# lastz/lastz

Measured on AMD Instinct MI355X. Metric: Gbp-of-target aligned/sec (whole job, --nogapped HSP path, both strands), higher is better.
Workload: dtype s32

## Files before the change

lastz_amd/csrc/enum_kernels.hip:

```cpp
#include <hip/hip_runtime.h>
#include <algorithm>
#include <rocprim/device/device_radix_sort.hpp>
#include <rocprim/device/device_scan.hpp>
#include <rocprim/iterator/transform_iterator.hpp>
#include "lz_ctx.hpp"
#include "lz_host.hpp"
#include "lz_seed_dev.hpp"

__global__ void __launch_bounds__(LZ_TPB)
k_pack_words(const u8* __restrict__ qcode, u32 lo, u32 hi, LzSeedDev sd, u32* __restrict__ pk, u32* __restrict__ iv, u32 bshift, u32 kbits)
{
    __shared__ u8 win[LZ_TPB + 32];
    const u32 i = blockIdx.x * LZ_TPB + threadIdx.x;
    const u32 L = (u32)sd.length;
    const s64 first = (s64)lo + (s64)blockIdx.x * LZ_TPB + 1 - (s64)L;
    for (u32 k = threadIdx.x; k < LZ_TPB + L - 1; k += LZ_TPB) win[k] = (first + (s64)k < (s64)hi) ? qcode[first + (s64)k] : (u8)LZ_CODE_INVALID;
    __syncthreads();
    if (i < hi - lo) {
        const u32 pos2 = lo + i + 1;
        u64 w = 0; u32 bad = 0;
        for (u32 k = 0; k < L; k++) { const u32 c = win[threadIdx.x + k]; bad |= c; w = (w << 2) | LZ_CODE_BITS(c); }
        const bool valid = pos2 >= lo + L && !(bad & LZ_CODE_INVALID);
        pk[i] = ((i >> bshift) << kbits) | (valid ? lz_apply_seed(sd, w) : (1u << sd.weight));
        iv[i] = i;
    }
}
__global__ void k_block_starts(const u32* __restrict__ sk, u32 n, u32 kbits, u32 none, u32 nblk, u64* __restrict__ bs, u64* __restrict__ n_words)
{
    const u32 b = threadIdx.x;
    if (b > nblk) return;
    auto first_at_least = [&](u64 key) { u32 lo = 0, hi = n; while (lo < hi) { const u32 m = lo + ((hi - lo) >> 1); if ((u64)sk[m] < key) lo = m + 1; else hi = m; } return lo; };
    const u32 start = first_at_least((u64)b << kbits);
    bs[b] = start;
    if (b < nblk) atomicAdd((unsigned long long*)n_words, (unsigned long long)(first_at_least(((u64)b << kbits) | none) - start));
}

__global__ void __launch_bounds__(LZ_TPB)
k_count_sorted(const u32* __restrict__ sk, const u32* __restrict__ sv, u32 n, LzSeedDev sd,
               const u32* __restrict__ wstart, u32* __restrict__ cnt)
{
    const u32 j = blockIdx.x * LZ_TPB + threadIdx.x;
    if (j >= n) return;
    const u32 w0 = sk[j] & ((2u << sd.weight) - 1u);
    if (w0 >> sd.weight) return;
    u32 c = 0;
    for (int p = 0; p < sd.nprobes; p++) { const u32 w = w0 ^ sd.probe_xor[p]; c += wstart[w + 1] - wstart[w]; }
    cnt[sv[j]] = c;
}

__device__ __forceinline__ bool lz_owned(u32 pos1, u32 pos2, u32 n_owners, u32 owner)
{ return (((pos1 - pos2) & (LZ_DIAG_SIZE - 1)) % n_owners) == owner; }

__global__ void __launch_bounds__(LZ_TPB)
k_count_sorted_owned(const u32* __restrict__ sk, const u32* __restrict__ sv, u32 n, u32 lo, LzSeedDev sd,
                     const u32* __restrict__ wstart, const u32* __restrict__ wpos, u32* __restrict__ cnt,
                     u32 n_owners, u32 owner)
{
    const u32 j = blockIdx.x * LZ_TPB + threadIdx.x;
    if (j >= n) return;
    const u32 w0 = sk[j] & ((2u << sd.weight) - 1u);
    if (w0 >> sd.weight) return;
    const u32 i = sv[j], pos2 = lo + i + 1;
    u32 c = 0;
    for (int p = 0; p < sd.nprobes; p++) {
        const u32 w = w0 ^ sd.probe_xor[p];
        for (u32 k = wstart[w]; k < wstart[w + 1]; k++) c += lz_owned(wpos[k], pos2, n_owners, owner) ? 1u : 0u;
    }
    cnt[i] = c;
}

#define LZ_SELF_GROUP 16
__global__ void __launch_bounds__(LZ_TPB)
k_count_sorted_self(const u32* __restrict__ sk, const u32* __restrict__ sv, u32 n, u32 lo, LzSeedDev sd,
                    const u32* __restrict__ wstart, const u32* __restrict__ wpos, u32* __restrict__ cnt, LzSelfDev self)
{
    const u32 j = blockIdx.x * LZ_TPB + threadIdx.x;
    if (j >= n) return;
    const u32 w0 = sk[j] & ((2u << sd.weight) - 1u);
    if (w0 >> sd.weight) return;
    const u32 i = sv[j], pos2 = lo + i + 1;
    u32 blo, bhi;
    lz_self_bounds(self, pos2, blo, bhi);
    u32 c = 0;
    for (int r = 0; r < sd.nprobes; r += LZ_SELF_GROUP) {
        u32 a[LZ_SELF_GROUP], len[LZ_SELF_GROUP];
#pragma unroll
        for (int p = 0; p < LZ_SELF_GROUP; p++) {
            const bool on = r + p < sd.nprobes;
            const u32 w = on ? (w0 ^ sd.probe_xor[(r + p) & (LZ_MAX_PROBES - 1)]) : 0u;
            a[p] = wstart[w]; len[p] = wstart[w + 1];
        }
#pragma unroll
        for (int p = 0; p < LZ_SELF_GROUP; p++) { const bool on = r + p < sd.nprobes; len[p] = on ? len[p] - a[p] : 0u; }
        lz_clip_runs<LZ_SELF_GROUP>(wpos, a, len, blo, bhi);
#pragma unroll
        for (int p = 0; p < LZ_SELF_GROUP; p++) c += len[p];
    }
    cnt[i] = c;
}

int lzk_count_hits(LzCtx& c, const u8* qcode, u32 lo, u32 hi)
{
    const u32 n = hi - lo;
    u32* const cnt = c.cnt.as<u32>(); u32* const pk = c.pk.as<u32>(); u32* const iv = c.wiv.as<u32>();
    u32* const sk = c.wsk.as<u32>(); u32* const sv = c.wsv.as<u32>();
    LZ_HIP(hipMemsetAsync(cnt, 0, (size_t)n * 4, c.stream));
    const u32 kbits = (u32)c.seed.weight + 1u;
    const double est_hits = (double)n * (double)c.num_words * (double)c.seed.nprobes / (double)(1ull << c.seed.weight);
    u32 want_bits = 0;
    while (want_bits < 5 && est_hits > (double)c.hit_capacity * (double)(1u << want_bits) * 0.5) want_bits++;
    if (est_hits <= (double)c.hit_capacity) want_bits = 0;
    u32 bbits = std::min<u32>(want_bits, 32u - kbits);
    u32 bshift = 0;
    const u64 nm1 = n ? (u64)n - 1 : 0;
    while (bshift < 32 && (nm1 >> bshift) >= (1ull << bbits)) bshift++;
    c.blk_shift = bshift; c.blk_count = (u32)((nm1 >> bshift) + 1);
    c.timer.begin("k_pack_words", c.stream);
    hipLaunchKernelGGL(k_pack_words, dim3((n + LZ_TPB - 1) / LZ_TPB), dim3(LZ_TPB), 0, c.stream,
                       qcode, lo, hi, c.seed, pk, iv, bshift, kbits);
    c.timer.end(c.stream);
    LZ_HIP(hipGetLastError());
    size_t tmp = 0;
    const unsigned bits = kbits + bbits;
    LZ_HIP(rocprim::radix_sort_pairs(nullptr, tmp, pk, sk, iv, sv, (size_t)n, 0u, bits, c.stream));
    int rc = c.sort_tmp.ensure(tmp);
    if (rc) return rc;
    c.timer.begin("rocprim_sort_words", c.stream);
    LZ_HIP(rocprim::radix_sort_pairs(c.sort_tmp.p, tmp, pk, sk, iv, sv, (size_t)n, 0u, bits, c.stream));
    c.timer.end(c.stream);
    if ((rc = c.blk_start.ensure(130 * 8))) return rc;
    hipLaunchKernelGGL(k_block_starts, dim3(1), dim3(192), 0, c.stream, sk, n, kbits, 1u << c.seed.weight, c.blk_count, c.blk_start.as<u64>(), c.dev_counters.as<u64>() + 2);
    c.timer.begin("k_count_hits", c.stream);
    if (c.self.mode != LZ_SELF_OFF)
        hipLaunchKernelGGL(k_count_sorted_self, dim3((n + LZ_TPB - 1) / LZ_TPB), dim3(LZ_TPB), 0, c.stream,
                           sk, sv, n, lo, c.seed, c.wstart.as<u32>(), c.wpos.as<u32>(), cnt, c.self);
    else if (c.n_owners > 1)
        hipLaunchKernelGGL(k_count_sorted_owned, dim3((n + LZ_TPB - 1) / LZ_TPB), dim3(LZ_TPB), 0, c.stream,
                           sk, sv, n, lo, c.seed, c.wstart.as<u32>(), c.wpos.as<u32>(), cnt, c.n_owners, c.owner);
    else
        hipLaunchKernelGGL(k_count_sorted, dim3((n + LZ_TPB - 1) / LZ_TPB), dim3(LZ_TPB), 0, c.stream,
                           sk, sv, n, c.seed, c.wstart.as<u32>(), cnt);
    c.timer.end(c.stream);
    LZ_HIP(hipGetLastError());
    return 0;
}

struct U32ToU64 { __host__ __device__ u64 operator()(u32 x) const { return (u64)x; } };

int lzk_scan_counts(LzCtx& c, u32 n)
{
    const u32* const cnt = c.cnt.as<u32>(); u64* const off = c.off.as<u64>();
    auto in = rocprim::make_transform_iterator(cnt, U32ToU64());
    size_t tmp = 0;
    LZ_HIP(rocprim::exclusive_scan(nullptr, tmp, in, off, (u64)0, (size_t)n, rocprim::plus<u64>(), c.stream));
    int rc = c.scan_tmp.ensure(tmp);
    if (rc) return rc;
    c.timer.begin("rocprim_scan_counts", c.stream);
    LZ_HIP(rocprim::exclusive_scan(c.scan_tmp.p, tmp, in, off, (u64)0, (size_t)n, rocprim::plus<u64>(), c.stream));
    c.timer.end(c.stream);
    return 0;
}

__global__ void __launch_bounds__(LZ_TPB)
k_sample_offsets(const u64* __restrict__ off, const u32* __restrict__ cnt, u32 n, u32 stride, u32 ns, u64* __restrict__ out)
{
    const u32 k = blockIdx.x * LZ_TPB + threadIdx.x;
    if (k < ns) out[1 + k] = off[(size_t)k * stride];
    if (k == 0) out[0] = off[n - 1] + cnt[n - 1];
}

int lzk_sample_offsets(LzCtx& c, u32 n, u32 stride, u32 ns)
{
    hipLaunchKernelGGL(k_sample_offsets, dim3((ns + LZ_TPB - 1) / LZ_TPB), dim3(LZ_TPB), 0, c.stream, c.off.as<u64>(), c.cnt.as<u32>(), n, stride, ns, c.pinned);
    LZ_HIP(hipGetLastError());
    return 0;
}

__global__ void __launch_bounds__(LZ_TPB)
k_fill_hits(u32 lo, u32 i0, u32 i1, LzSeedDev sd,
            const u32* __restrict__ wstart, const u32* __restrict__ wpos,
            const u32* __restrict__ sk, const u32* __restrict__ sv, u32 n, const u64* __restrict__ off,
            u64 base, u64* __restrict__ keys, u32 n_owners, u32 owner)
{
    const u32 lane = threadIdx.x & 63u, p = lane & (LZ_FILL_GROUP - 1), g = lane >> 4;
    const u32 j = (blockIdx.x * LZ_TPB + threadIdx.x);
    u32 w_l = 0, i_l = 0; bool in = false;
    if (j < n) { w_l = sk[j] & ((2u << sd.weight) - 1u); i_l = sv[j]; in = !(w_l >> sd.weight) && i_l >= i0 && i_l < i1; }
    u64 todo = __ballot(in);
    while (todo) {
        int src = -1;
        u64 m = todo;
#pragma unroll
        for (int q = 0; q < 4; q++) {
            const int s_q = m ? (int)__ffsll((long long)m) - 1 : -1;
            if (m) m &= m - 1;
            if ((int)g == q) src = s_q;
        }
        todo = m;
        const bool have = src >= 0;
        const u32 packed = __shfl(w_l, have ? src : 0);
        const u32 i = __shfl(i_l, have ? src : 0);
        const u32 pos2 = lo + i + 1;
        u64* out = have ? keys + (off[i] - base) : keys;
        u32 carry = 0;
        for (int r = 0; r < sd.nprobes; r += LZ_FILL_GROUP) {
            u32 a = 0, len = 0, full = 0;
            if (have && r + (int)p < sd.nprobes) {
                const u32 w = packed ^ sd.probe_xor[r + p];
                a = wstart[w]; full = wstart[w + 1] - a;
                for (u32 jj = 0; jj < full; jj++) len += lz_owned(wpos[a + jj], pos2, n_owners, owner) ? 1u : 0u;
            }
            u32 incl = len;
#pragma unroll
            for (int d = 1; d < LZ_FILL_GROUP; d <<= 1) {
                u32 v = __shfl_up(incl, d, LZ_FILL_GROUP);
                if ((int)p >= d) incl += v;
            }
            const u32 total = __shfl(incl, LZ_FILL_GROUP - 1, LZ_FILL_GROUP);
            u64* o = out + carry + (incl - len);
            for (u32 jj = 0; jj < full; jj++) { const u32 p1 = wpos[a + jj]; if (lz_owned(p1, pos2, n_owners, owner)) *o++ = lz_hit_key(p1, pos2); }
            carry += total;
        }
    }
}

#define LZ_F2_CAP   2560
#define LZ_F2_WORDS (LZ_F2_CAP / 2 / 64)
template <bool SELF>
__global__ void __launch_bounds__(LZ_TPB)
k_fill_hits2(u32 lo, u32 i0, u32 i1, LzSeedDev sd,
             const u32* __restrict__ wstart, const u32* __restrict__ wpos,
             const u32* __restrict__ sk, const u32* __restrict__ sv, u32 n, const u64* __restrict__ off,
             u64 base, u64* __restrict__ keys, LzSelfDev self)
{
    __shared__ LzListWave<LZ_F2_CAP> shw[LZ_TPB / 64];
    LzListWave<LZ_F2_CAP>& sh = shw[threadIdx.x >> 6];
    unsigned short* const own = reinterpret_cast<unsigned short*>(sh.own32);
    const u32 lane = threadIdx.x & 63u;
    const u32 j = blockIdx.x * LZ_TPB + threadIdx.x;
    u32 w_l = 0, i_l = 0; bool in = false;
    if (j < n) { w_l = sk[j] & ((2u << sd.weight) - 1u); i_l = sv[j]; in = !(w_l >> sd.weight) && i_l >= i0 && i_l < i1; }
    if (!__ballot(in)) return;
    const u32 dbase = in ? (u32)(off[i_l] - base) : 0u;
    const u32 pos2 = lo + i_l + 1u;
    u32 slo = 0, shi = 0;
    if (SELF) lz_self_bounds(self, pos2, slo, shi);
    u32 carry = 0;
    for (int r = 0; r < sd.nprobes; r += LZ_FILL_GROUP) {
        u32 la[LZ_FILL_GROUP], len[LZ_FILL_GROUP]; u32 total = 0;
#pragma unroll
        for (int p = 0; p < LZ_FILL_GROUP; p++) {
            const bool on = in && r + p < sd.nprobes;
            const u32 w = on ? (w_l ^ sd.probe_xor[(r + p) & (LZ_MAX_PROBES - 1)]) : 0u;
            la[p] = wstart[w]; len[p] = wstart[w + 1];
        }
#pragma unroll
        for (int p = 0; p < LZ_FILL_GROUP; p++) {
            const bool on = in && r + p < sd.nprobes;
            len[p] = on ? len[p] - la[p] : 0u;
            if (!SELF) total += len[p];
        }
        if (SELF) {
            lz_clip_runs<LZ_FILL_GROUP>(wpos, la, len, slo, shi);
#pragma unroll
            for (int p = 0; p < LZ_FILL_GROUP; p++) total += len[p];
        }
        u32 inc = total;
        LZ_WAVE_SCAN_U32(inc, total, lz_uadd)
        const u32 E = inc - total;
        const u32 T = (u32)__builtin_amdgcn_readlane((int)inc, 63);
        {
            u32 S = E;
#pragma unroll
            for (int p = 0; p < LZ_FILL_GROUP; p++) { sh.lsrc[lane * LZ_FILL_GROUP + p] = la[p] - S; S += len[p]; }
        }
        sh.ent[lane] = make_uint2(dbase + carry - E, pos2);
        for (u32 cs = 0; cs < T; cs += LZ_F2_CAP) {
            const u32 tc = (T - cs < (u32)LZ_F2_CAP) ? T - cs : (u32)LZ_F2_CAP;
            uint4* const mine = reinterpret_cast<uint4*>(sh.own32 + lane * LZ_F2_WORDS);
#pragma unroll
            for (int k = 0; k < LZ_F2_WORDS / 4; k++) mine[k] = make_uint4(0u, 0u, 0u, 0u);
            __atomic_signal_fence(__ATOMIC_SEQ_CST);
            {
                u32 S = E;
#pragma unroll
                for (int p = 0; p < LZ_FILL_GROUP; p++) {
                    const u32 l = len[p];
                    if (l && S < cs + tc && S + l > cs) own[(S > cs ? S : cs) - cs] = (unsigned short)(1u + lane * LZ_FILL_GROUP + (u32)p);
                    S += l;
                }
            }
            __atomic_signal_fence(__ATOMIC_SEQ_CST);
            u32 wv[LZ_F2_WORDS];
#pragma unroll
// ... 61 lines not shown
```

lastz_amd/csrc/lz_ctx.hpp:

```cpp
#pragma once
#include <hip/hip_runtime.h>
#include <string>
#include <vector>
#include <map>
#include <mutex>
#include "lz_common.hpp"
#include "lz_settings.hpp"
#include "../../include/lzgpu.h"

struct DevBuf {
    void*  p = nullptr;
    size_t cap = 0;
    int ensure(size_t bytes);
    void release();
    template <class T> T* as() const { return (T*)p; }
};

struct KernelTimer {
    struct Pending { int id; hipEvent_t a, b; hipStream_t s; };
    bool enabled = false;
    std::vector<std::string> names;
    std::vector<uint64_t> launches;
    std::vector<double> ms;
    std::vector<Pending> pending;
    std::map<hipStream_t, std::vector<hipEvent_t>> pool;
    int  id_of(const char* name);
    void begin(const char* name, hipStream_t s);
    void end(hipStream_t s);
    void resolve();
    void reset();
    hipEvent_t get_event(hipStream_t s);
    int cur = -1; hipEvent_t cur_a = nullptr;
};

struct SeqSlot {
    DevBuf raw;
    DevBuf code;
    DevBuf dp;
    DevBuf nib;
    bool   have_nib = false;
    DevBuf two, spc;
    DevBuf two_x, spc_x;
    DevBuf occ_dev;
    u8     occ[256] = { 0 };
    bool   has_special = false;
    u32    len = 0;
    bool   have_raw = false;
    uint64_t code_key = 0;
    uint64_t dp_key = 0;
    std::vector<u8> host;
    u8* raw_base()  const { return raw.as<u8>()  + LZ_SEQ_PAD; }
    u8* code_base() const { return code.as<u8>() + LZ_SEQ_PAD; }
    void release()
    {
        DevBuf* all[] = { &raw, &code, &dp, &nib, &two, &spc, &two_x, &spc_x, &occ_dev };
        for (DevBuf* b : all) b->release();
        have_raw = have_nib = false; code_key = dp_key = 0;
    }
};

struct LzCtx {
    bool inited = false;
    int  device = -1;
    int  num_cus = 256;
    hipStream_t stream = nullptr;
    hipStream_t dp_stream = nullptr;
    std::string last_error;

    SeqSlot target;
    bool have_table = false;
    lz_table_geom geom;
    LzSeedDev seed;
    DevBuf wstart, wpos;
    u64 num_words = 0;
    u64 table_gen = 0;
    DevBuf wctx;
    u64 wctx_gen = 0; uint64_t wctx_code_key = 0;

    std::map<int, SeqSlot> queries;
#define LZ_TEMP_SLOT_B3 (-1000)
    std::mutex slots_m;

    DevBuf cnt, off, pk;
    DevBuf wiv, wsk, wsv;
    DevBuf blk_start;
    std::vector<u64> blk_start_host;
    u32 blk_shift = 0, blk_count = 1;
    u64* pinned = nullptr; size_t pinned_words = 0;
    DevBuf bins;
    DevBuf keys;
    DevBuf bin_base;
    DevBuf hist, hist_part, run_addr;
    DevBuf summ, scan_tasks, scan_ntasks;
    DevBuf lut;
    DevBuf sort_tmp, scan_tmp;
    DevBuf diag_end;
    DevBuf score_tab;
    std::vector<s32> score_sub;
    u8 rowc[256] = { 0 }, colc[256] = { 0 };
    std::vector<s32> lut_m4; s32 lut_xdrop = -1;
    DevBuf cls_t, cls_q, cls_tmp;
    DevBuf win_tab;
    DevBuf hsp_out, hsp_count;
    DevBuf hsp_mc;
    DevBuf dev_counters;
    DevBuf tb_keys, tb_vals, tb_keys2, tb_vals2;
    struct DpBufs { DevBuf jobs, ids, res, tab, tb, rows, ops, ops_off, ops_out, pieces, rings, sel_jobs, sel_res, problems; } dp;
    DevBuf win_jobs, win_scratch, win_out, win_count;
    bool win_attr_set = false;
    bool settle_attr_set = false;
    u64 dp_longest[4] = { 0, 0, 0, 0 };
    u32 dp_slot_tb = 8u << 20;
    u32 dp_window = 0;
    u32 n_owners = 1, owner = 0;
    LzSelfDev self = {};
    DevBuf self_sep;
    std::vector<u64> last_order;
    int min_scan_mode = 0;
    int last_scan_mode = -1;
    u64 hit_capacity = (1ull << 31);
    u64 hsp_capacity = (1ull << 24);

    lz_counters counters = {};
    std::mutex counters_m;
    KernelTimer timer;
    KernelTimer dp_timer;

    void release_device_memory()
    {
        DevBuf* all[] = { &wstart, &wpos, &wctx, &cnt, &off, &pk, &wiv, &wsk, &wsv, &blk_start, &bins, &keys, &bin_base, &hist, &hist_part, &run_addr,
                          &summ, &scan_tasks, &scan_ntasks, &lut, &sort_tmp, &scan_tmp, &diag_end, &score_tab, &cls_t, &cls_q, &cls_tmp, &win_tab,
                          &hsp_out, &hsp_count, &hsp_mc, &dev_counters, &tb_keys, &tb_vals, &tb_keys2, &tb_vals2, &self_sep,
                          &dp.jobs, &dp.ids, &dp.res, &dp.tab, &dp.tb, &dp.rows, &dp.ops, &dp.ops_off, &dp.ops_out, &dp.pieces, &dp.rings, &dp.sel_jobs, &dp.sel_res, &dp.problems,
                          &win_jobs, &win_scratch, &win_out, &win_count };
        for (DevBuf* b : all) b->release();
        target.release();
        for (auto& kv : queries) kv.second.release();
        queries.clear();
        if (pinned) (void)hipHostFree(pinned);
        pinned = nullptr; pinned_words = 0;
        have_table = false; wctx_gen = 0; wctx_code_key = 0;
        score_sub.clear(); lut_m4.clear(); lut_xdrop = -1;
        win_attr_set = false; settle_attr_set = false;
    }
};

LzCtx& lz_ctx();
int lz_bind_thread();
int lz_fail(int code, const char* fmt, ...);
#define LZ_HIP(expr) do { hipError_t _e = (expr); if (_e != hipSuccess) \
    return lz_fail(LZGPU_ERR_HIP, "%s:%d %s -> %s", __FILE__, __LINE__, #expr, hipGetErrorString(_e)); } while (0)

struct LzChunk; struct LzLutParams;
#include "lz_tile_runs.hpp"
int lzk_encode(LzCtx& c, const u8* raw, u8* code, u32 len, const u8* cls256_dev, hipStream_t st = nullptr, KernelTimer* timer = nullptr);
int lzk_pack_nibbles(LzCtx& c, const u8* code_alloc, u8* nib, size_t nbytes);
int lzk_pack2(LzCtx& c, const u8* code_base, const u8* raw_base, u32 len, u8* two, u8* spc, u32 nmask, u32* flags256);
int lzk_overlap32(LzCtx& c, const u8* src, u8* dst, size_t nblocks);
int lzk_table_build(LzCtx& c);
int lzk_table_export(LzCtx& c, u32* last_dev, u32* prev_dev, u32 prev_entries);
int lzk_wctx_build(LzCtx& c);
int lzk_count_hits(LzCtx& c, const u8* qcode, u32 lo, u32 hi);
int lzk_scan_counts(LzCtx& c, u32 n);
int lzk_sample_offsets(LzCtx& c, u32 n, u32 stride, u32 ns);
int lzk_fill_hits(LzCtx& c, u32 lo, const LzChunk& ch, u32 n);
int lzk_scan_reserve(LzCtx& c, int mode, u64 max_n);
int lzk_scan_hits(LzCtx& c, int mode, const LzExtendParams& P, const LzLutParams& Q, u64 n);
int lzk_fused_reserve(LzCtx& c, u64 max_n);
int lzk_scan_fused(LzCtx& c, u32 lo, const LzChunk& ch, u32 n, const LzExtendParams& P, const LzLutParams& Q);
int lzk_partition(LzCtx& c, bool tagged, u64 n);
int lzk_hist_scan(LzCtx& c, u64 n);
int lzk_settle(LzCtx& c, const LzExtendParams& P, u64 n, u32 out_cap);
int lzk_hsp_match_counts(LzCtx& c, u32 n_rec, const SeqSlot& q);
```

lastz_amd/csrc/lzgpu_api.hip:

```cpp
#include <hip/hip_runtime.h>
#include <stdarg.h>
#include <stdio.h>
#include <stdlib.h>
#include <string.h>
#include <math.h>
#include <algorithm>
#include <mutex>
#include <thread>
#include <atomic>
#include "lz_ctx.hpp"
#include "lz_host.hpp"
#include "lz_lut.hpp"


static LzCtx g_ctx;
void lz_phase_clocks_print();
LzCtx& lz_ctx() { return g_ctx; }

static thread_local std::string t_last_error, t_last_error_out;
static std::mutex g_err_m;
int lz_fail(int code, const char* fmt, ...)
{
    char buf[512];
    va_list ap; va_start(ap, fmt); vsnprintf(buf, sizeof(buf), fmt, ap); va_end(ap);
// ... 281 lines not shown
    memset(&c.geom, 0, sizeof(c.geom));
    c.geom.tlen = tlen; c.geom.start = start; c.geom.end = end; c.geom.step = step; c.geom.seed = *seed;
    memcpy(c.geom.char_to_bits, char_to_bits, 256);
    if ((rc = slot_upload(c, c.target, t, tlen, true))) return rc;
    u8 cls[256]; lzh_make_cls(nullptr, char_to_bits, cls);
    if ((rc = slot_encode(c, c.target, cls, c.cls_t))) return rc;
    if ((rc = lzk_table_build(c))) return rc;
    c.geom.num_words = c.num_words;
    c.have_table = true;
    return 0;
}

extern "C" int lzgpu_target_upload(const uint8_t* t, uint32_t tlen)
{
    int rc = require_init(); if (rc) return rc;
    LzCtx& c = g_ctx;
    if (!t) return lz_fail(LZGPU_ERR_ARG, "null argument");
    if (tlen >= 0x7FFFFFFFu) return LZGPU_NH_SIZE;
    c.have_table = false;
    memset(&c.geom, 0, sizeof(c.geom));
    c.geom.tlen = tlen;
    return slot_upload(c, c.target, t, tlen, true);
}

extern "C" int lzgpu_table_rebuild(void)
{
    LzCtx& c = g_ctx;
    if (!c.have_table) return lz_fail(LZGPU_ERR_STATE, "no position table");
    int rc = lz_bind_thread(); if (rc) return rc;
    rc = lzk_table_build(c);
    if (!rc) c.geom.num_words = c.num_words;
    return rc;
}

extern "C" uint64_t lzgpu_table_num_words(void) { return g_ctx.have_table ? g_ctx.num_words : 0; }

extern "C" int lzgpu_table_export(uint32_t* last, uint32_t* prev)
{
    LzCtx& c = g_ctx;
    if (!c.have_table) return lz_fail(LZGPU_ERR_STATE, "no position table");
    u32 nwords = 1u << c.seed.weight;
    u32 adj = c.geom.start - (c.geom.start % c.geom.step);
    u32 prev_entries = 1 + (c.geom.end - adj) / c.geom.step;
    DevBuf dl, dp; int rc;
    if ((rc = lz_bind_thread())) return rc;
    if (last && (rc = dl.ensure((size_t)nwords * 4))) return rc;
    if (prev && (rc = dp.ensure((size_t)prev_entries * 4))) { dl.release(); return rc; }
    rc = lzk_table_export(c, last ? dl.as<u32>() : nullptr, prev ? dp.as<u32>() : nullptr, prev_entries);
    if (!rc) {
        if (last) (void)hipMemcpyAsync(last, dl.p, (size_t)nwords * 4, hipMemcpyDeviceToHost, c.stream);
        if (prev) (void)hipMemcpyAsync(prev, dp.p, (size_t)prev_entries * 4, hipMemcpyDeviceToHost, c.stream);
        if (hipStreamSynchronize(c.stream) != hipSuccess) rc = lz_fail(LZGPU_ERR_HIP, "table export copy failed");
    }
    dl.release(); dp.release();
    return rc;
}

extern "C" int lzgpu_table_geom(lz_table_geom* out)
{
    if (!g_ctx.have_table || !out) return lz_fail(LZGPU_ERR_STATE, "no position table");
    *out = g_ctx.geom; return 0;
}

extern "C" int lzgpu_table_adopt(const lz_table_geom* g)
{
    int rc = require_init(); if (rc) return rc;
    LzCtx& c = g_ctx;
    if (!g) return LZGPU_ERR_ARG;
    if ((rc = lzh_seed_to_dev(&g->seed, c.seed))) return rc;
    c.have_table = false; c.geom = *g; c.num_words = g->num_words; c.table_gen++;
    size_t total = (size_t)g->tlen + 2 * LZ_SEQ_PAD + 16;
    if ((rc = c.target.raw.ensure(total))) return rc;
    if ((rc = c.target.code.ensure(total))) return rc;
    LZ_HIP(hipMemsetAsync(c.target.raw.p, 0, total, c.stream));
    LZ_HIP(hipMemsetAsync(c.target.code.p, LZ_CODE_INVALID, total, c.stream));
    c.target.len = g->tlen; c.target.have_raw = true; c.target.code_key = 0; c.target.dp_key = 0; c.target.host.clear();
    if ((rc = c.wstart.ensure(((size_t)(1u << c.seed.weight) + 1) * 4))) return rc;
    if ((rc = c.wpos.ensure((size_t)(g->num_words ? g->num_words : 1) * 4))) return rc;
    LZ_HIP(hipStreamSynchronize(c.stream));
    return 0;
}

extern "C" int lzgpu_table_buffers(void* dev_ptr[3], uint64_t bytes[3])
{
    LzCtx& c = g_ctx;
    if (!c.target.have_raw || !c.wstart.p) return lz_fail(LZGPU_ERR_STATE, "no table buffers");
    dev_ptr[0] = c.target.raw_base(); bytes[0] = c.geom.tlen;
    dev_ptr[1] = c.wstart.p;          bytes[1] = ((uint64_t)(1u << c.seed.weight) + 1) * 4;
    dev_ptr[2] = c.wpos.p;            bytes[2] = (uint64_t)c.num_words * 4;
    return 0;
}

extern "C" int lzgpu_table_commit(void)
{
    LzCtx& c = g_ctx;
    if (!c.target.have_raw || !c.wstart.p) return lz_fail(LZGPU_ERR_STATE, "no table buffers");
    { int rc = lz_bind_thread(); if (rc) return rc; }
    if (c.target.host.size() != c.geom.tlen) {
        c.target.host.resize(c.geom.tlen);
        if (c.geom.tlen) LZ_HIP(hipMemcpy(c.target.host.data(), c.target.raw_base(), c.geom.tlen, hipMemcpyDeviceToHost));
        c.target.code_key = 0; c.target.dp_key = 0;
    }
    c.table_gen++;
    c.have_table = true;
    return 0;
}

extern "C" int lzgpu_device_copy(void* dst, const void* src, uint64_t bytes)
{
    int rc = require_init(); if (rc) return rc;
    if (!bytes) return 0;
    LZ_HIP(hipMemcpyAsync(dst, src, bytes, hipMemcpyDeviceToDevice, g_ctx.stream));
    LZ_HIP(hipStreamSynchronize(g_ctx.stream));
    return 0;
}


#include <chrono>
struct HostProf {
    bool on = false; double t[16]; const char* names[16] = { nullptr }; int n = 0;
    std::chrono::steady_clock::time_point last;
    HostProf() { for (auto& x : t) x = 0; }
    void start() { on = lz_settings().hostprof; if (on) last = std::chrono::steady_clock::now(); }
    void lap(int k, const char* name) {
        if (!on) return;
        auto now = std::chrono::steady_clock::now();
        t[k] += std::chrono::duration<double, std::milli>(now - last).count(); names[k] = name; if (k >= n) n = k + 1; last = now;
    }
    ~HostProf() { if (on) for (int k = 0; k < n; k++) if (names[k]) fprintf(stderr, "[lzgpu hostprof] %-28s %10.2f ms total\n", names[k], t[k]); }
};
static HostProf g_hp;

static int lz_wctx_prepare(LzCtx& c, bool& fused)
{
    if (c.wctx.p && c.wctx_gen == c.table_gen && c.wctx_code_key == c.target.code_key && c.target.code_key) return 0;
    const size_t need = (size_t)c.num_words * LZ_WCTX_BYTES;
    if (c.num_words == 0) { fused = false; return 0; }
    if (need > c.wctx.cap || !c.wctx.p) {
        size_t fr = 0, tot = 0;
        if (hipMemGetInfo(&fr, &tot) != hipSuccess || need > (fr + c.wctx.cap) / 2 || c.wctx.ensure(need) != 0) {
            (void)hipGetLastError(); c.last_error.clear();
            c.wctx_gen = 0; c.wctx_code_key = 0;
            fused = false;
            return 0;
        }
    }
    c.wctx_gen = 0; c.wctx_code_key = 0;
    int rc = lzk_wctx_build(c);
    if (rc) return rc;
    c.wctx_gen = c.table_gen; c.wctx_code_key = c.target.code_key;
    return 0;
}

static int lz_search_query(LzCtx& c, const u8* bytes, u32 len, int slot, bool upload, SeqSlot*& qs, u32& qlen)
{
    qs = nullptr; qlen = len;
    if (bytes) {
        if (!upload) return 0;
        if (len >= 0x7FFFFFFFu) return LZGPU_NH_SIZE;
        qs = lz_query_slot(c, -1, true);
        return slot_upload(c, *qs, bytes, len, false);
    }
    qs = slot < 0 ? nullptr : lz_query_slot(c, slot, false);
    if (!qs) return lz_fail(LZGPU_ERR_ARG, "query slot %d is empty", slot);
    qlen = qs->len;
    return 0;
}

static int lz_hsps_out(const std::vector<lz_hsp>& v, lz_hsp** out, uint64_t* n_out)
{
    lz_hsp* res = (lz_hsp*)malloc((v.size() ? v.size() : 1) * sizeof(lz_hsp));
    if (!res) return lz_fail(LZGPU_ERR_OOM, "host malloc failed");
    if (!v.empty()) memcpy(res, v.data(), v.size() * sizeof(lz_hsp));
    *out = res; *n_out = v.size();
    return 0;
}

static int search_enter(bool args_ok, lz_hsp** out, uint64_t* n_out)
{
    int rc = require_init(); if (rc) return rc;
    if (!args_ok) return lz_fail(LZGPU_ERR_ARG, "null argument");
    *out = nullptr; *n_out = 0;
    if (!g_ctx.have_table) return lz_fail(LZGPU_ERR_STATE, "lzgpu_table_prepare has not been called");
    return 0;
}

struct SeedSearch {
    const lz_search_args* a;
    SeqSlot* qs = nullptr; const u8* qhost = nullptr;
    u32 lo = 0, hi = 0, n = 0, L = 0;
    u64 total_hits = 0;
    std::vector<LzChunk> chunks; u64 max_chunk = 0;
    int mode = 2; bool fused = false;
    LzExtendParams P; LzLutParams Q;
    u32 out_cap = 0;
    std::vector<lz_hsp> plain;
};

static int ss_query(LzCtx& c, SeedSearch& s)
{
    const lz_search_args* a = s.a;
    u32 qlen;
    int rc = lz_search_query(c, a->query, a->qlen, a->query_slot, true, s.qs, qlen); if (rc) return rc;
    s.qhost = a->query ? a->query : s.qs->host.data();
    s.lo = a->start; s.hi = a->end ? a->end : qlen;
    if (s.hi <= s.lo) return lz_fail(LZGPU_ERR_ARG, "in seed_hit_search(), interval is void (%u-%u)", s.lo, s.hi);
    if (s.hi > qlen) return lz_fail(LZGPU_ERR_ARG, "in seed_hit_search(), interval end is bad (%u>%u)", s.hi, qlen);
    s.n = s.hi - s.lo; s.L = (u32)c.seed.length;
    g_hp.lap(7, "query slot");
    return 0;
}

static int ss_classes(LzCtx& c, SeedSearch& s)
{
    const s32* sub = s.a->sub;
    int rc;
    if (c.score_sub.size() != 65536 || memcmp(c.score_sub.data(), sub, 65536 * sizeof(s32)) != 0) {
        s32 tab[LZ_NCLASS * LZ_NCLASS];
        c.score_sub.clear();
        if ((rc = lzh_score_classes(sub, c.rowc, c.colc, tab))) return rc;
        if ((rc = c.score_tab.ensure(sizeof(tab)))) return rc;
        LZ_HIP(hipMemcpyAsync(c.score_tab.p, tab, sizeof(tab), hipMemcpyHostToDevice, c.stream));
        LZ_HIP(hipStreamSynchronize(c.stream));
        c.score_sub.assign(sub, sub + 65536);
    }
    g_hp.lap(8, "score classes + table upload");
    u8 cls[256];
    lzh_make_cls(c.rowc, c.geom.char_to_bits, cls);
    if ((rc = slot_encode(c, c.target, cls, c.cls_t))) return rc;
    lzh_make_cls(c.colc, c.geom.char_to_bits, cls);
    if ((rc = slot_encode(c, *s.qs, cls, c.cls_q))) return rc;
    g_hp.lap(0, "upload+classes+encode");
    return 0;
}

static const u32 LZ_PLAN_STRIDE = 4096;
static int ss_count(LzCtx& c, SeedSearch& s)
{
    const u32 n = s.n;
    int rc;
    if ((rc = c.cnt.ensure((size_t)n * 4))) return rc;
    if ((rc = c.off.ensure((size_t)n * 8))) return rc;
    if ((rc = c.pk.ensure((size_t)n * 4))) return rc;
    if ((rc = c.wiv.ensure((size_t)n * 4))) return rc;
    if ((rc = c.wsk.ensure((size_t)n * 4))) return rc;
    if ((rc = c.wsv.ensure((size_t)n * 4))) return rc;
    if ((rc = c.diag_end.ensure((size_t)LZ_DIAG_SIZE * 4))) return rc;
    if ((rc = c.dev_counters.ensure(8 * 8))) return rc;
    if ((rc = c.hsp_count.ensure(4))) return rc;
    LZ_HIP(hipMemsetAsync(c.diag_end.p, 0, (size_t)LZ_DIAG_SIZE * 4, c.stream));
    LZ_HIP(hipMemsetAsync(c.dev_counters.p, 0, 64, c.stream));
    LZ_HIP(hipMemsetAsync(c.hsp_count.p, 0, 4, c.stream));

    if ((rc = lzk_count_hits(c, s.qs->code_base(), s.lo, s.hi))) return rc;
    if ((rc = lzk_scan_counts(c, n))) return rc;

    const u32 ns = (n + LZ_PLAN_STRIDE - 1) / LZ_PLAN_STRIDE;
    if (c.pinned_words < (size_t)ns + 16) {
        if (c.pinned) (void)hipHostFree(c.pinned);
        c.pinned = nullptr; c.pinned_words = 0;
        LZ_HIP(hipHostMalloc((void**)&c.pinned, ((size_t)ns + 16) * 8, hipHostMallocDefault));
        c.pinned_words = (size_t)ns + 16;
    }
    if ((rc = lzk_sample_offsets(c, n, LZ_PLAN_STRIDE, ns))) return rc;
    c.blk_start_host.assign((size_t)c.blk_count + 1, 0);
    LZ_HIP(hipMemcpyAsync(c.blk_start_host.data(), c.blk_start.p, ((size_t)c.blk_count + 1) * 8, hipMemcpyDeviceToHost, c.stream));
    LZ_HIP(hipStreamSynchronize(c.stream));
    g_hp.lap(1, "count+scan (sync)");
    c.timer.resolve();
    s.total_hits = c.pinned[0];
    return 0;
}

static int ss_plan(LzCtx& c, SeedSearch& s)
{
    const u64* samp = c.pinned + 1;
    hipError_t fetch_err = hipSuccess;
    auto off_at = [&](u32 i) -> u64 {
        if (i >= s.n) return s.total_hits;
        if (i % LZ_PLAN_STRIDE == 0) return samp[i / LZ_PLAN_STRIDE];
        u64 v = 0;
        hipError_t e = hipMemcpy(&v, c.off.as<u64>() + i, 8, hipMemcpyDeviceToHost);
        if (e != hipSuccess) fetch_err = e;
        return v;
    };
    int rc = lzh_plan_chunks(s.n, c.hit_capacity, LZ_PLAN_STRIDE, off_at, s.chunks); if (rc) return rc;
    if (fetch_err != hipSuccess) return lz_fail(LZGPU_ERR_HIP, "prefix fetch failed: %s", hipGetErrorString(fetch_err));
    for (auto& ch : s.chunks) if (ch.nh > s.max_chunk) s.max_chunk = ch.nh;
    g_hp.lap(2, "chunk plan");
    return 0;
}

static int ss_scan_mode(LzCtx& c, SeedSearch& s)
{
    const lz_search_args* a = s.a;
    SeqSlot* qs = s.qs;
    LzExtendParams& P = s.P; LzLutParams& Q = s.Q;
    P.tcode = c.target.code_base(); P.tlen = c.geom.tlen;
    P.qcode = qs->code_base();      P.qlen = qs->len;
    P.xdrop = a->xdrop; P.min_score = a->hsp_threshold; P.seed_len = s.L;
    P.cls8 = lzh_small_classes(c.rowc, c.colc);
    const bool nibs = P.cls8 && c.target.have_nib && qs->have_nib;
    P.tnib = nibs ? c.target.nib.as<u8>() : nullptr; P.qnib = nibs ? qs->nib.as<u8>() : nullptr;
    Q.t2 = c.target.two.as<u8>(); Q.q2 = qs->two.as<u8>(); Q.tsp = c.target.spc.as<u8>(); Q.qsp = qs->spc.as<u8>(); Q.xdrop = a->xdrop;
    Q.t2x = c.target.two_x.as<u8>(); Q.tspx = c.target.spc_x.as<u8>();
    Q.tcode = P.tcode; Q.qcode = P.qcode;

    int mode = 2, rc;
    if (a->extend) {
        s32 M4[16];
        if (lzh_lut_eligible(a->sub, c.geom.char_to_bits, c.target.occ, qs->occ, a->xdrop, M4))
            mode = (c.target.has_special || qs->has_special) ? 1 : 0;
        if (mode < c.min_scan_mode) mode = c.min_scan_mode;
        if (mode < 2 && (c.lut_xdrop != a->xdrop || c.lut_m4.size() != 16 || memcmp(c.lut_m4.data(), M4, sizeof(M4)) != 0)) {
            std::vector<LzLutEntry> lut_host(LZ_LUT_TOTAL);
            c.lut_m4.clear();
            lzh_lut_build(M4, a->xdrop, lut_host.data());
            if ((rc = c.lut.ensure(lut_host.size() * sizeof(LzLutEntry)))) return rc;
            LZ_HIP(hipMemcpyAsync(c.lut.p, lut_host.data(), lut_host.size() * sizeof(LzLutEntry), hipMemcpyHostToDevice, c.stream));
            LZ_HIP(hipStreamSynchronize(c.stream));
            c.lut_m4.assign(M4, M4 + 16); c.lut_xdrop = a->xdrop;
        }
    }
    s.mode = c.last_scan_mode = mode;
    s.fused = a->extend && mode == 0 && s.max_chunk && lz_settings().fused_scan && c.n_owners <= 1;
    if (s.fused && (rc = lz_wctx_prepare(c, s.fused))) return rc;
    return 0;
}

static int ss_reserve(LzCtx& c, SeedSearch& s)
{
    const bool extend = s.a->extend != 0;
    const u64 max_chunk = s.max_chunk;
    int rc;
    if (max_chunk) {
        if ((rc = c.keys.ensure((size_t)max_chunk * 8))) return rc;
        if (!s.fused && (rc = c.bins.ensure((size_t)max_chunk + 64))) return rc;
    }
    if (extend && max_chunk) {
        const size_t ntiles = (size_t)((max_chunk + LZ_PP_TILE_HOST - 1) / LZ_PP_TILE_HOST), nblocks = (ntiles + 255) / 256;
        if ((rc = c.bin_base.ensure(257 * 4))) return rc;
        if ((rc = c.hist.ensure(ntiles * 256 * 4))) return rc;
        if ((rc = c.hist_part.ensure(nblocks * 256 * 4))) return rc;
        if ((rc = c.run_addr.ensure(ntiles * 256 * 4))) return rc;
    }
    s.out_cap = (u32)std::min<u64>(c.hsp_capacity, 0xFFFFFFF0ull);
    if (extend && (rc = c.hsp_out.ensure((size_t)s.out_cap * sizeof(LzHspRec)))) return rc;
    if (extend && max_chunk && (rc = s.fused ? lzk_fused_reserve(c, max_chunk) : lzk_scan_reserve(c, s.mode, max_chunk))) return rc;
    return 0;
}

static int ss_chunk(LzCtx& c, SeedSearch& s, const LzChunk& ch)
{
    int rc;
    if (s.fused) {
        if ((rc = lzk_scan_fused(c, s.lo, ch, s.n, s.P, s.Q))) return rc;
    } else {
        if ((rc = lzk_fill_hits(c, s.lo, ch, s.n))) return rc;
        if ((rc = lzk_scan_hits(c, s.mode, s.P, s.Q, ch.nh))) return rc;
    }
    if ((rc = lzk_partition(c, s.fused, ch.nh))) return rc;
    if ((rc = lzk_hist_scan(c, ch.nh))) return rc;
    return lzk_settle(c, s.P, ch.nh, s.out_cap);
}
static int ss_chunk_plain(LzCtx& c, SeedSearch& s, const LzChunk& ch)
{
    int rc = lzk_fill_hits(c, s.lo, ch, s.n); if (rc) return rc;
    std::vector<u64> hk(ch.nh);
    LZ_HIP(hipMemcpyAsync(hk.data(), c.keys.p, (size_t)ch.nh * 8, hipMemcpyDeviceToHost, c.stream));
    LZ_HIP(hipStreamSynchronize(c.stream));
    for (u64 k : hk) { u32 p2 = (u32)k; s.plain.push_back({ p2 + (u32)(k >> 32), p2, s.L, 0 }); }
    return 0;
}

static int ss_finish(LzCtx& c, SeedSearch& s, lz_hsp** out, uint64_t* n_out)
{
    const lz_search_args* a = s.a;
    int rc;
    u64 hc[3] = { 0, 0, 0 }; u32 n_rec = 0;
    LZ_HIP(hipMemcpyAsync(hc, c.dev_counters.p, 24, hipMemcpyDeviceToHost, c.stream));
    LZ_HIP(hipMemcpyAsync(&n_rec, c.hsp_count.p, 4, hipMemcpyDeviceToHost, c.stream));
    LZ_HIP(hipStreamSynchronize(c.stream));
    g_hp.lap(4, "wait for GPU");
    const bool gpu_counts = a->extend && n_rec > 0 && n_rec <= s.out_cap;
    if (gpu_counts) {
        if ((rc = c.hsp_mc.ensure((size_t)n_rec * 20))) return rc;
        if ((rc = lzk_hsp_match_counts(c, n_rec, *s.qs))) return rc;
    }
    c.timer.resolve();
    { std::lock_guard<std::mutex> lk(c.counters_m);
      c.counters.words += hc[2]; c.counters.raw_hits += s.total_hits;
      c.counters.extensions += hc[0]; c.counters.bp_extended += hc[1]; }
    if (!a->extend) return lz_hsps_out(s.plain, out, n_out);
    if (n_rec > s.out_cap) return LZGPU_NH_HSP_OVERFLOW;

    std::vector<LzHspRec> recs(n_rec);
    std::vector<u32> mc;
    if (n_rec) LZ_HIP(hipMemcpyAsync(recs.data(), c.hsp_out.p, (size_t)n_rec * sizeof(LzHspRec), hipMemcpyDeviceToHost, c.stream));
    if (gpu_counts) { mc.resize((size_t)n_rec * 5); LZ_HIP(hipMemcpyAsync(mc.data(), c.hsp_mc.p, (size_t)n_rec * 20, hipMemcpyDeviceToHost, c.stream)); }
    LZ_HIP(hipStreamSynchronize(c.stream));
    c.timer.resolve();
    g_hp.lap(5, "copy candidates");
    std::vector<lz_hsp> fin;
    if ((rc = lzh_finish_hsps(recs.data(), n_rec, c.target.host.data(), s.qhost, c.seed, c.geom.char_to_bits,
                              a->hsp_threshold, a->entropic, fin, gpu_counts ? mc.data() : nullptr, &c.last_order)))
        return lz_fail(rc, "internal: candidate HSP is not on a seed hit");
// ... 146 lines not shown
```

lastz_amd/csrc/table_kernels.hip:

```cpp
#include <hip/hip_runtime.h>
#include <rocprim/device/device_radix_sort.hpp>
#include "lz_ctx.hpp"
#include "lz_lut.hpp"
#include "lz_seed_dev.hpp"

__global__ void __launch_bounds__(LZ_TPB)
k_table_words(const u8* __restrict__ tcode, u32 start, u32 end, u32 step, LzSeedDev sd,
              u32* __restrict__ keys, u32* __restrict__ vals, u32 n)
{
    u32 j = blockIdx.x * LZ_TPB + threadIdx.x;
    if (j >= n) return;
    u32 p = end - j;
    u32 key = 1u << sd.weight;
    if (p >= start + (u32)sd.length && (p % step) == 0) {
        u32 packed;
        if (lz_window_word(tcode, p, sd, packed)) key = packed;
    }
    keys[j] = key; vals[j] = p;
}

__global__ void __launch_bounds__(LZ_TPB)
k_key_bounds_u32(const u32* __restrict__ keys, u32 n, u32 nwords, u32* __restrict__ wstart)
{
    u32 i = blockIdx.x * LZ_TPB + threadIdx.x;
    if (i > n) return;
    s64 kp = (i == 0) ? -1 : (s64)keys[i - 1];
    s64 k  = (i == n) ? (s64)nwords : (s64)keys[i];
    if (k > (s64)nwords) k = nwords;
    if (kp > (s64)nwords) kp = nwords;
    for (s64 w = kp + 1; w <= k; w++) wstart[w] = i;
}

int lzk_table_build(LzCtx& c)
{
    const lz_table_geom& g = c.geom;
    const u32 n = g.end - g.start;
    const u32 nwords = 1u << c.seed.weight;
    int rc;
    if ((rc = c.tb_keys.ensure((size_t)n * 4))) return rc;
    if ((rc = c.tb_vals.ensure((size_t)n * 4))) return rc;
    if ((rc = c.tb_keys2.ensure((size_t)n * 4))) return rc;
    if ((rc = c.tb_vals2.ensure((size_t)n * 4))) return rc;
    if ((rc = c.wstart.ensure(((size_t)nwords + 1) * 4))) return rc;

    c.timer.begin("k_table_words", c.stream);
    hipLaunchKernelGGL(k_table_words, dim3((n + LZ_TPB - 1) / LZ_TPB), dim3(LZ_TPB), 0, c.stream,
                       c.target.code_base(), g.start, g.end, g.step, c.seed,
                       c.tb_keys.as<u32>(), c.tb_vals.as<u32>(), n);
    c.timer.end(c.stream);
    LZ_HIP(hipGetLastError());

    size_t tmp = 0;
    LZ_HIP(rocprim::radix_sort_pairs(nullptr, tmp, c.tb_keys.as<u32>(), c.tb_keys2.as<u32>(),
                                     c.tb_vals.as<u32>(), c.tb_vals2.as<u32>(), (size_t)n, 0u,
                                     (unsigned)c.seed.weight + 1u, c.stream));
    if ((rc = c.sort_tmp.ensure(tmp))) return rc;
    c.timer.begin("rocprim_sort_table", c.stream);
    LZ_HIP(rocprim::radix_sort_pairs(c.sort_tmp.p, tmp, c.tb_keys.as<u32>(), c.tb_keys2.as<u32>(),
                                     c.tb_vals.as<u32>(), c.tb_vals2.as<u32>(), (size_t)n, 0u,
                                     (unsigned)c.seed.weight + 1u, c.stream));
    c.timer.end(c.stream);

    c.timer.begin("k_key_bounds_u32", c.stream);
    hipLaunchKernelGGL(k_key_bounds_u32, dim3((n + 1 + LZ_TPB - 1) / LZ_TPB), dim3(LZ_TPB), 0, c.stream,
                       c.tb_keys2.as<u32>(), n, nwords, c.wstart.as<u32>());
    c.timer.end(c.stream);
    LZ_HIP(hipGetLastError());

    u32 nw = 0;
    LZ_HIP(hipMemcpyAsync(&nw, c.wstart.as<u32>() + nwords, 4, hipMemcpyDeviceToHost, c.stream));
    LZ_HIP(hipStreamSynchronize(c.stream));
    c.timer.resolve();
    c.num_words = nw;
    c.table_gen++;
    if ((rc = c.wpos.ensure((size_t)(nw ? nw : 1) * 4))) return rc;
    LZ_HIP(hipMemcpyAsync(c.wpos.p, c.tb_vals2.p, (size_t)nw * 4, hipMemcpyDeviceToDevice, c.stream));
    LZ_HIP(hipStreamSynchronize(c.stream));
    return 0;
}

__global__ void __launch_bounds__(LZ_TPB)
k_table_export(const u32* __restrict__ wstart, const u32* __restrict__ wpos, u32 nwords,
               u32 adj_start, u32 step, u32* __restrict__ last, u32* __restrict__ prev)
{
    u32 w = blockIdx.x * LZ_TPB + threadIdx.x;
    if (w >= nwords) return;
    u32 a = wstart[w], b = wstart[w + 1];
    if (a == b) return;
    if (last) last[w] = (wpos[a] - adj_start) / step;
    if (prev)
        for (u32 j = a; j < b; j++)
            prev[(wpos[j] - adj_start) / step] = (j + 1 < b) ? (wpos[j + 1] - adj_start) / step : 0xFFFFFFFFu;
}

int lzk_table_export(LzCtx& c, u32* last_dev, u32* prev_dev, u32 prev_entries)
{
    const u32 nwords = 1u << c.seed.weight;
    if (last_dev) LZ_HIP(hipMemsetAsync(last_dev, 0, (size_t)nwords * 4, c.stream));
    if (prev_dev) LZ_HIP(hipMemsetAsync(prev_dev, 0, (size_t)prev_entries * 4, c.stream));
    u32 adj = c.geom.start - (c.geom.start % c.geom.step);
    hipLaunchKernelGGL(k_table_export, dim3((nwords + LZ_TPB - 1) / LZ_TPB), dim3(LZ_TPB), 0, c.stream,
                       c.wstart.as<u32>(), c.wpos.as<u32>(), nwords, adj, c.geom.step, last_dev, prev_dev);
    LZ_HIP(hipGetLastError());
    return 0;
}

__global__ void __launch_bounds__(LZ_TPB)
k_build_wctx(const u32* __restrict__ wpos, u64 num_words, const u8* __restrict__ two, LzVec16* __restrict__ wctx)
{
    const u64 j = (u64)blockIdx.x * LZ_TPB + threadIdx.x;
    if (j >= 2 * num_words) return;
    const u32 pos1 = wpos[j >> 1];
    wctx[j] = lz_load16(two + lz_wctx_first_byte(pos1) + 16u * (u32)(j & 1u));
}

int lzk_wctx_build(LzCtx& c)
{
    const u64 nw = c.num_words;
    if (nw == 0) return 0;
    c.timer.begin("k_build_wctx", c.stream);
    hipLaunchKernelGGL(k_build_wctx, dim3((unsigned)((2 * nw + LZ_TPB - 1) / LZ_TPB)), dim3(LZ_TPB), 0, c.stream,
                       c.wpos.as<u32>(), nw, c.target.two.as<u8>(), c.wctx.as<LzVec16>());
    c.timer.end(c.stream);
    LZ_HIP(hipGetLastError());
    return 0;
}
```

Baseline: 0.4074.

## Precompute per-word hit counts and fuse counting into word packing kernel

Adds a per-table word-count array, built once per table generation, that sums probe-run lengths for each seed word. In the default non-self, single-owner path the pack kernel now writes per-position hit counts directly, which removes the separate count kernel, the memset, and the random gathers through the sorted values. Valid-word counting moves into the pack kernel through a wave scan plus atomic, so the block-starts kernel needs only one binary search. The pack kernel becomes grid-stride with a capped grid, the sort skips an unneeded key bit when there is no block bucketing, and the table build swaps buffers instead of copying and synchronising. The cost is an extra table-sized array and its build kernel.

After: 0.4154, median of 6. 1.02x the previous value.

```diff
diff --git a/lastz_amd/csrc/enum_kernels.hip b/lastz_amd/csrc/enum_kernels.hip
--- a/lastz_amd/csrc/enum_kernels.hip
+++ b/lastz_amd/csrc/enum_kernels.hip
@@ -7,45 +7,52 @@
 #include "lz_host.hpp"
 #include "lz_seed_dev.hpp"
 
-__global__ void __launch_bounds__(LZ_TPB)
-k_pack_words(const u8* __restrict__ qcode, u32 lo, u32 hi, LzSeedDev sd, u32* __restrict__ pk, u32* __restrict__ iv, u32 bshift, u32 kbits)
+template <bool COUNT>
+__global__ void __launch_bounds__(LZ_TPB)
+k_pack_words(const u8* __restrict__ qcode, u32 lo, u32 hi, LzSeedDev sd, u32* __restrict__ pk, u32* __restrict__ iv, u32 bshift, u32 kbits,
+             const u32* __restrict__ wcnt, u32* __restrict__ cnt, u64* __restrict__ n_words)
 {
     __shared__ u8 win[LZ_TPB + 32];
-    const u32 i = blockIdx.x * LZ_TPB + threadIdx.x;
+    __shared__ u32 nvalid[LZ_TPB / 64];
     const u32 L = (u32)sd.length;
-    const s64 first = (s64)lo + (s64)blockIdx.x * LZ_TPB + 1 - (s64)L;
-    for (u32 k = threadIdx.x; k < LZ_TPB + L - 1; k += LZ_TPB) win[k] = (first + (s64)k < (s64)hi) ? qcode[first + (s64)k] : (u8)LZ_CODE_INVALID;
+    const u32 ntiles = (hi - lo + LZ_TPB - 1) / LZ_TPB;
+    u32 mine = 0;
+    for (u32 tile = blockIdx.x; tile < ntiles; tile += gridDim.x) {
+        const u32 i = tile * LZ_TPB + threadIdx.x;
+        const s64 first = (s64)lo + (s64)tile * LZ_TPB + 1 - (s64)L;
+        for (u32 k = threadIdx.x; k < LZ_TPB + L - 1; k += LZ_TPB) win[k] = (first + (s64)k < (s64)hi) ? qcode[first + (s64)k] : (u8)LZ_CODE_INVALID;
+        __syncthreads();
+        if (i < hi - lo) {
+            const u32 pos2 = lo + i + 1;
+            u64 w = 0; u32 bad = 0;
+            for (u32 k = 0; k < L; k++) { const u32 c = win[threadIdx.x + k]; bad |= c; w = (w << 2) | LZ_CODE_BITS(c); }
+            const bool valid = pos2 >= lo + L && !(bad & LZ_CODE_INVALID);
+            const u32 word = valid ? lz_apply_seed(sd, w) : (1u << sd.weight);
+            pk[i] = ((i >> bshift) << kbits) | word;
+            iv[i] = i;
+            if (COUNT) cnt[i] = valid ? wcnt[word] : 0u;
+            mine += valid ? 1u : 0u;
+        }
+        __syncthreads();
+    }
+    u32 inc = mine;
+    LZ_WAVE_SCAN_U32(inc, mine, lz_uadd)
+    if ((threadIdx.x & 63u) == 63u) nvalid[threadIdx.x >> 6] = inc;
     __syncthreads();
-    if (i < hi - lo) {
-        const u32 pos2 = lo + i + 1;
-        u64 w = 0; u32 bad = 0;
-        for (u32 k = 0; k < L; k++) { const u32 c = win[threadIdx.x + k]; bad |= c; w = (w << 2) | LZ_CODE_BITS(c); }
-        const bool valid = pos2 >= lo + L && !(bad & LZ_CODE_INVALID);
-        pk[i] = ((i >> bshift) << kbits) | (valid ? lz_apply_seed(sd, w) : (1u << sd.weight));
-        iv[i] = i;
-    }
-}
-__global__ void k_block_starts(const u32* __restrict__ sk, u32 n, u32 kbits, u32 none, u32 nblk, u64* __restrict__ bs, u64* __restrict__ n_words)
+    if (threadIdx.x == 0) {
+        u32 t = 0;
+        for (u32 k = 0; k < LZ_TPB / 64; k++) t += nvalid[k];
+        if (t) atomicAdd((unsigned long long*)n_words, (unsigned long long)t);
+    }
+}
+__global__ void k_block_starts(const u32* __restrict__ sk, u32 n, u32 kbits, u32 nblk, u64* __restrict__ bs)
 {
     const u32 b = threadIdx.x;
     if (b > nblk) return;
-    auto first_at_least = [&](u64 key) { u32 lo = 0, hi = n; while (lo < hi) { const u32 m = lo + ((hi - lo) >> 1); if ((u64)sk[m] < key) lo = m + 1; else hi = m; } return lo; };
-    const u32 start = first_at_least((u64)b << kbits);
-    bs[b] = start;
-    if (b < nblk) atomicAdd((unsigned long long*)n_words, (unsigned long long)(first_at_least(((u64)b << kbits) | none) - start));
-}
-
-__global__ void __launch_bounds__(LZ_TPB)
-k_count_sorted(const u32* __restrict__ sk, const u32* __restrict__ sv, u32 n, LzSeedDev sd,
-               const u32* __restrict__ wstart, u32* __restrict__ cnt)
-{
-    const u32 j = blockIdx.x * LZ_TPB + threadIdx.x;
-    if (j >= n) return;
-    const u32 w0 = sk[j] & ((2u << sd.weight) - 1u);
-    if (w0 >> sd.weight) return;
-    u32 c = 0;
-    for (int p = 0; p < sd.nprobes; p++) { const u32 w = w0 ^ sd.probe_xor[p]; c += wstart[w + 1] - wstart[w]; }
-    cnt[sv[j]] = c;
+    const u64 key = (u64)b << kbits;
+    u32 lo = 0, hi = n;
+    while (lo < hi) { const u32 m = lo + ((hi - lo) >> 1); if ((u64)sk[m] < key) lo = m + 1; else hi = m; }
+    bs[b] = lo;
 }
 
 __device__ __forceinline__ bool lz_owned(u32 pos1, u32 pos2, u32 n_owners, u32 owner)
@@ -104,7 +111,8 @@
     const u32 n = hi - lo;
     u32* const cnt = c.cnt.as<u32>(); u32* const pk = c.pk.as<u32>(); u32* const iv = c.wiv.as<u32>();
     u32* const sk = c.wsk.as<u32>(); u32* const sv = c.wsv.as<u32>();
-    LZ_HIP(hipMemsetAsync(cnt, 0, (size_t)n * 4, c.stream));
+    u64* const n_words = c.dev_counters.as<u64>() + 2;
+    const bool by_word = c.self.mode == LZ_SELF_OFF && c.n_owners <= 1;
     const u32 kbits = (u32)c.seed.weight + 1u;
     const double est_hits = (double)n * (double)c.num_words * (double)c.seed.nprobes / (double)(1ull << c.seed.weight);
     u32 want_bits = 0;
@@ -115,13 +123,19 @@
     const u64 nm1 = n ? (u64)n - 1 : 0;
     while (bshift < 32 && (nm1 >> bshift) >= (1ull << bbits)) bshift++;
     c.blk_shift = bshift; c.blk_count = (u32)((nm1 >> bshift) + 1);
-    c.timer.begin("k_pack_words", c.stream);
-    hipLaunchKernelGGL(k_pack_words, dim3((n + LZ_TPB - 1) / LZ_TPB), dim3(LZ_TPB), 0, c.stream,
-                       qcode, lo, hi, c.seed, pk, iv, bshift, kbits);
+    const dim3 grid((n + LZ_TPB - 1) / LZ_TPB);
+    const dim3 pack_grid(std::min<u32>(grid.x, (u32)c.num_cus * 8u));
+    if (by_word) {
+        c.timer.begin("k_count_hits", c.stream);
+        hipLaunchKernelGGL(k_pack_words<true>, pack_grid, dim3(LZ_TPB), 0, c.stream, qcode, lo, hi, c.seed, pk, iv, bshift, kbits, c.wcnt.as<u32>(), cnt, n_words);
+    } else {
+        c.timer.begin("k_pack_words", c.stream);
+        hipLaunchKernelGGL(k_pack_words<false>, pack_grid, dim3(LZ_TPB), 0, c.stream, qcode, lo, hi, c.seed, pk, iv, bshift, kbits, nullptr, nullptr, n_words);
+    }
     c.timer.end(c.stream);
     LZ_HIP(hipGetLastError());
+    const unsigned bits = bbits ? kbits + bbits : kbits - 1u;
     size_t tmp = 0;
-    const unsigned bits = kbits + bbits;
     LZ_HIP(rocprim::radix_sort_pairs(nullptr, tmp, pk, sk, iv, sv, (size_t)n, 0u, bits, c.stream));
     int rc = c.sort_tmp.ensure(tmp);
     if (rc) return rc;
@@ -129,17 +143,16 @@
     LZ_HIP(rocprim::radix_sort_pairs(c.sort_tmp.p, tmp, pk, sk, iv, sv, (size_t)n, 0u, bits, c.stream));
     c.timer.end(c.stream);
     if ((rc = c.blk_start.ensure(130 * 8))) return rc;
-    hipLaunchKernelGGL(k_block_starts, dim3(1), dim3(192), 0, c.stream, sk, n, kbits, 1u << c.seed.weight, c.blk_count, c.blk_start.as<u64>(), c.dev_counters.as<u64>() + 2);
+    hipLaunchKernelGGL(k_block_starts, dim3(1), dim3(192), 0, c.stream, sk, n, kbits, c.blk_count, c.blk_start.as<u64>());
+    if (by_word) return 0;
+    LZ_HIP(hipMemsetAsync(cnt, 0, (size_t)n * 4, c.stream));
     c.timer.begin("k_count_hits", c.stream);
     if (c.self.mode != LZ_SELF_OFF)
-        hipLaunchKernelGGL(k_count_sorted_self, dim3((n + LZ_TPB - 1) / LZ_TPB), dim3(LZ_TPB), 0, c.stream,
+        hipLaunchKernelGGL(k_count_sorted_self, grid, dim3(LZ_TPB), 0, c.stream,
                            sk, sv, n, lo, c.seed, c.wstart.as<u32>(), c.wpos.as<u32>(), cnt, c.self);
-    else if (c.n_owners > 1)
-        hipLaunchKernelGGL(k_count_sorted_owned, dim3((n + LZ_TPB - 1) / LZ_TPB), dim3(LZ_TPB), 0, c.stream,
+    else
+        hipLaunchKernelGGL(k_count_sorted_owned, grid, dim3(LZ_TPB), 0, c.stream,
                            sk, sv, n, lo, c.seed, c.wstart.as<u32>(), c.wpos.as<u32>(), cnt, c.n_owners, c.owner);
-    else
-        hipLaunchKernelGGL(k_count_sorted, dim3((n + LZ_TPB - 1) / LZ_TPB), dim3(LZ_TPB), 0, c.stream,
-                           sk, sv, n, c.seed, c.wstart.as<u32>(), cnt);
     c.timer.end(c.stream);
     LZ_HIP(hipGetLastError());
     return 0;
diff --git a/lastz_amd/csrc/lz_ctx.hpp b/lastz_amd/csrc/lz_ctx.hpp
--- a/lastz_amd/csrc/lz_ctx.hpp
+++ b/lastz_amd/csrc/lz_ctx.hpp
@@ -76,6 +76,8 @@
     u64 table_gen = 0;
     DevBuf wctx;
     u64 wctx_gen = 0; uint64_t wctx_code_key = 0;
+    DevBuf wcnt;
+    u64 wcnt_gen = 0;
 
     std::map<int, SeqSlot> queries;
 #define LZ_TEMP_SLOT_B3 (-1000)
@@ -128,7 +130,7 @@
 
     void release_device_memory()
     {
-        DevBuf* all[] = { &wstart, &wpos, &wctx, &cnt, &off, &pk, &wiv, &wsk, &wsv, &blk_start, &bins, &keys, &bin_base, &hist, &hist_part, &run_addr,
+        DevBuf* all[] = { &wstart, &wpos, &wctx, &wcnt, &cnt, &off, &pk, &wiv, &wsk, &wsv, &blk_start, &bins, &keys, &bin_base, &hist, &hist_part, &run_addr,
                           &summ, &scan_tasks, &scan_ntasks, &lut, &sort_tmp, &scan_tmp, &diag_end, &score_tab, &cls_t, &cls_q, &cls_tmp, &win_tab,
                           &hsp_out, &hsp_count, &hsp_mc, &dev_counters, &tb_keys, &tb_vals, &tb_keys2, &tb_vals2, &self_sep,
                           &dp.jobs, &dp.ids, &dp.res, &dp.tab, &dp.tb, &dp.rows, &dp.ops, &dp.ops_off, &dp.ops_out, &dp.pieces, &dp.rings, &dp.sel_jobs, &dp.sel_res, &dp.problems,
@@ -139,7 +141,7 @@
         queries.clear();
         if (pinned) (void)hipHostFree(pinned);
         pinned = nullptr; pinned_words = 0;
-        have_table = false; wctx_gen = 0; wctx_code_key = 0;
+        have_table = false; wctx_gen = 0; wctx_code_key = 0; wcnt_gen = 0;
         score_sub.clear(); lut_m4.clear(); lut_xdrop = -1;
         win_attr_set = false; settle_attr_set = false;
     }
@@ -160,6 +162,7 @@
 int lzk_table_build(LzCtx& c);
 int lzk_table_export(LzCtx& c, u32* last_dev, u32* prev_dev, u32 prev_entries);
 int lzk_wctx_build(LzCtx& c);
+int lzk_word_counts(LzCtx& c);
 int lzk_count_hits(LzCtx& c, const u8* qcode, u32 lo, u32 hi);
 int lzk_scan_counts(LzCtx& c, u32 n);
 int lzk_sample_offsets(LzCtx& c, u32 n, u32 stride, u32 ns);
diff --git a/lastz_amd/csrc/lzgpu_api.hip b/lastz_amd/csrc/lzgpu_api.hip
--- a/lastz_amd/csrc/lzgpu_api.hip
+++ b/lastz_amd/csrc/lzgpu_api.hip
@@ -457,6 +457,17 @@
     return 0;
 }
 
+static int lz_wcnt_prepare(LzCtx& c)
+{
+    if (c.wcnt.p && c.wcnt_gen == c.table_gen) return 0;
+    c.wcnt_gen = 0;
+    int rc = c.wcnt.ensure((size_t)(1u << c.seed.weight) * 4);
+    if (rc) return rc;
+    if ((rc = lzk_word_counts(c))) return rc;
+    c.wcnt_gen = c.table_gen;
+    return 0;
+}
+
 static int lz_search_query(LzCtx& c, const u8* bytes, u32 len, int slot, bool upload, SeqSlot*& qs, u32& qlen)
 {
     qs = nullptr; qlen = len;
@@ -557,6 +568,7 @@
     LZ_HIP(hipMemsetAsync(c.dev_counters.p, 0, 64, c.stream));
     LZ_HIP(hipMemsetAsync(c.hsp_count.p, 0, 4, c.stream));
 
+    if (c.self.mode == LZ_SELF_OFF && c.n_owners <= 1 && (rc = lz_wcnt_prepare(c))) return rc;
     if ((rc = lzk_count_hits(c, s.qs->code_base(), s.lo, s.hi))) return rc;
     if ((rc = lzk_scan_counts(c, n))) return rc;
 
diff --git a/lastz_amd/csrc/table_kernels.hip b/lastz_amd/csrc/table_kernels.hip
--- a/lastz_amd/csrc/table_kernels.hip
+++ b/lastz_amd/csrc/table_kernels.hip
@@ -1,4 +1,5 @@
 #include <hip/hip_runtime.h>
+#include <utility>
 #include <rocprim/device/device_radix_sort.hpp>
 #include "lz_ctx.hpp"
 #include "lz_lut.hpp"
@@ -73,9 +74,28 @@
     c.timer.resolve();
     c.num_words = nw;
     c.table_gen++;
-    if ((rc = c.wpos.ensure((size_t)(nw ? nw : 1) * 4))) return rc;
-    LZ_HIP(hipMemcpyAsync(c.wpos.p, c.tb_vals2.p, (size_t)nw * 4, hipMemcpyDeviceToDevice, c.stream));
-    LZ_HIP(hipStreamSynchronize(c.stream));
+    std::swap(c.wpos, c.tb_vals2);
+    return 0;
+}
+
+__global__ void __launch_bounds__(LZ_TPB)
+k_word_counts(const u32* __restrict__ wstart, LzSeedDev sd, u32 nwords, u32* __restrict__ wcnt)
+{
+    const u32 w0 = blockIdx.x * LZ_TPB + threadIdx.x;
+    if (w0 >= nwords) return;
+    u32 c = 0;
+    for (int p = 0; p < sd.nprobes; p++) { const u32 w = w0 ^ sd.probe_xor[p]; c += wstart[w + 1] - wstart[w]; }
+    wcnt[w0] = c;
+}
+
+int lzk_word_counts(LzCtx& c)
+{
+    const u32 nwords = 1u << c.seed.weight;
+    c.timer.begin("k_word_counts", c.stream);
+    hipLaunchKernelGGL(k_word_counts, dim3((nwords + LZ_TPB - 1) / LZ_TPB), dim3(LZ_TPB), 0, c.stream,
+                       c.wstart.as<u32>(), c.seed, nwords, c.wcnt.as<u32>());
+    c.timer.end(c.stream);
+    LZ_HIP(hipGetLastError());
     return 0;
 }
 
```
